# Da-Tsuchi/KLab_MultiModalModel

Hardware: AMD Instinct MI355X
Metric: caption-train samples/sec (224px img, 64-tok tgt) (higher is better)
Workload: dtype bf16; 1 GPU; BASELINE configs[1]: Swin-V2(C=64,(2,2,6,2),224,w7) frozen + T5-small, fwd+bwd+Adam, T5 dropout 0.1 on, random-init weights; global_batch=64, per_gpu_batch=64, src_len=9, tgt_len=64, parallelism=dp1, hipgraph=False, optimizer=klab.optim.FusedAdam (Adam update of ref/train.py:28, one kernel)

## Files before the change

include/klab_mm.h:

```cpp
#ifndef KLAB_MM_H
#define KLAB_MM_H
#include <stddef.h>
#include <stdint.h>

#ifdef __cplusplus
extern "C" {
#endif

#define KLAB_OK 0
#define KLAB_ERR_UNSUPPORTED (-2)
#define KLAB_ERR_BADARG (-3)

#define KLAB_F32 0
#define KLAB_BF16 1
#define KLAB_FP8 2

#define KLAB_ACT_NONE 0
#define KLAB_ACT_RELU 1
#define KLAB_ACT_GELU 2

#define KLAB_AUX_NONE 0
#define KLAB_AUX_NONZERO 1
#define KLAB_AUX_DGELU 2

// ... 54 lines not shown
                            int grp_stride, int off, float drop_p, const uint32_t* seed_dev, uint32_t tag, void* stream);

typedef struct klab_attn_args {
  int dtype;
  const void* q; long ldq;
  const void* k; long ldk;
  const void* v; long ldv;
  const float* bias; int causal;
  void* ctx; long ldo;
  float* lse;
  int B, H, Lq, Lk, dk;
  float drop_p; const uint32_t* seed_dev; uint32_t drop_tag;
  const void* dctx; long lddo;
  void* dq; long lddq;
  void* dk_out; long lddk;
  void* dv; long lddv;
  float* dbias;
  void* ds_ws;
  int ds_defer;
  const float* score_scale;
  int bias_mod;
} klab_attn_args;
int klab_t5_attn_fwd(const klab_attn_args* a, void* stream);
int klab_t5_attn_bwd(const klab_attn_args* a, void* stream);
typedef struct klab_attn_fused_args {
  const float* x; const float* gamma; float eps; int d_model;
  const void* w;
  void* xn; float* rstd;
  void* proj; long ldproj;
  int cross;
  klab_attn_args attn;
} klab_attn_fused_args;
int klab_t5_attn_fused_fwd(const klab_attn_fused_args* a, void* stream);
int klab_dbias_reduce(const void* ds_ws, int dtype, float* dbias, int nbatch, int H, int Lq, int Lk, void* stream);

typedef struct klab_swin_attn_args {
  int dtype;
  const void* qkv; void* ctx; const float* bias; const float* logit_scale; float* lse;
  int B, R, w, shift, H, C;
  const void* dctx; void* dqkv; float* dbias; float* dlogit_scale;
  void* bwd_ws; size_t bwd_ws_bytes;
  const float* bias_table; float* dbias_table;
  const float* v_bias; float* dv_bias;
} klab_swin_attn_args;
int klab_swin_attn_fwd(const klab_swin_attn_args* a, void* stream);
size_t klab_swin_attn_bwd_ws_bytes(int dtype, int B, int R, int w, int H, int C);
int klab_swin_qkv_attn_fused(const void* x, const void* wqkv, const float* bqkv, void* ctx, const float* bias, const float* logit_scale,
                             int dtype, int B, int R, int w, int shift, int H, int C, void* stream);
int klab_swin_attn_bwd(const klab_swin_attn_args* a, void* stream);
int klab_swin_cpb_bias(const float* coords, const int* index, const float* w0, const float* b0, const float* w2,
                       float* table, float* hidden, float* bias, int ntab, int n, int heads, int nhidden, void* stream);
int klab_swin_cpb_table(const float* coords, const float* w0, const float* b0, const float* w2, float* table, float* hidden,
                        float* bias_table, int ntab, int heads, int nhidden, void* stream);
int klab_swin_cpb_table_bwd(const float* dbias_table, const float* bias_table, const float* coords, const float* hidden, const float* w2,
                            float* dtable, float* dw0, float* db0, float* dw2, int ntab, int heads, int nhidden, void* stream);

typedef struct klab_image_desc { long long offset; int height, width; } klab_image_desc;
size_t klab_image_preprocess_ws_bytes(int n_images, int max_h, int mid);
int klab_image_preprocess(const unsigned char* src, const klab_image_desc* desc_dev, int n_images, int max_h, int max_w, int mid,
                          int out_size, int filter_a, int filter_b, double rescale, const float* mean3, const float* std3,
                          float* pixel_values, void* ws, size_t ws_bytes, void* stream);

#define KLAB_JPEG_GRAY 0
#define KLAB_JPEG_YCC 1
#define KLAB_JPEG_RGB 2
typedef struct klab_jpeg_info {
// ... 151 lines not shown
```

klab_multimodalmodel_amd/_lib.py:

```python
import ctypes as C
import os

HERE = os.path.dirname(os.path.abspath(__file__))
LIB_PATH = os.environ.get("KLAB_LIB", os.path.join(HERE, "libklab_mm.so"))

F32, BF16, FP8 = 0, 1, 2
ACT_NONE, ACT_RELU, ACT_GELU = 0, 1, 2
AUX_NONE, AUX_NONZERO, AUX_DGELU = 0, 1, 2
ERR_UNSUPPORTED, ERR_BADARG = -2, -3

vp, i32, i64, f32, u32 = C.c_void_p, C.c_int, C.c_long, C.c_float, C.c_uint32


class GemmArgs(C.Structure):
    _fields_ = [("M", i32), ("N", i32), ("K", i32), ("dtype", i32),
                ("A", vp), ("lda", i64), ("a_kmajor", i32),
                ("B", vp), ("ldb", i64), ("b_kmajor", i32),
                ("C", vp), ("ldc", i64), ("c_dtype", i32), ("accumulate", i32),
                ("alpha", f32), ("alpha_dev", vp), ("bias", vp), ("act", i32),
                ("aux", vp), ("ldaux", i64), ("aux_mode", i32), ("aux_scale", f32),
                ("residual", vp), ("ldr", i64), ("r_dtype", i32),
                ("drop_p", f32), ("seed_dev", vp), ("drop_tag", u32), ("name_tag", i32), ("atomic_ok", i32)]


class AttnArgs(C.Structure):
    _fields_ = [("dtype", i32), ("q", vp), ("ldq", i64), ("k", vp), ("ldk", i64), ("v", vp), ("ldv", i64),
                ("bias", vp), ("causal", i32), ("ctx", vp), ("ldo", i64), ("lse", vp),
                ("B", i32), ("H", i32), ("Lq", i32), ("Lk", i32), ("dk", i32),
                ("drop_p", f32), ("seed_dev", vp), ("drop_tag", u32),
                ("dctx", vp), ("lddo", i64), ("dq", vp), ("lddq", i64), ("dk_out", vp), ("lddk", i64),
                ("dv", vp), ("lddv", i64), ("dbias", vp), ("ds_ws", vp), ("ds_defer", i32),
                ("score_scale", vp), ("bias_mod", i32)]


class AttnFusedArgs(C.Structure):
    _fields_ = [("x", vp), ("gamma", vp), ("eps", f32), ("d_model", i32), ("w", vp), ("xn", vp), ("rstd", vp), ("proj", vp), ("ldproj", i64),
                ("cross", i32), ("attn", AttnArgs)]


class SwinAttnArgs(C.Structure):
    _fields_ = [("dtype", i32), ("qkv", vp), ("ctx", vp), ("bias", vp), ("logit_scale", vp), ("lse", vp),
                ("B", i32), ("R", i32), ("w", i32), ("shift", i32), ("H", i32), ("C", i32),
                ("dctx", vp), ("dqkv", vp), ("dbias", vp), ("dlogit_scale", vp),
                ("bwd_ws", vp), ("bwd_ws_bytes", C.c_size_t), ("bias_table", vp), ("dbias_table", vp),
                ("v_bias", vp), ("dv_bias", vp)]


class BeamUpdateArgs(C.Structure):
    _fields_ = [("B", i32), ("k", i32), ("V", i32), ("max_length", i32), ("eos_id", i32), ("early_stopping", i32), ("length_penalty", f32),
                ("cand_score", vp), ("cand_idx", vp), ("run_seq_in", vp), ("run_seq_out", vp), ("run_score", vp),
                ("fin_seq_in", vp), ("fin_seq_out", vp), ("fin_score", vp), ("fin_flag", vp), ("fin_len", vp), ("unsat", vp),
                ("slot_in", vp), ("slot_out", vp), ("prev_tokens", vp), ("parent", vp), ("stop_word", vp)]


SIGNATURES = {
    "klab_version": [],
    "klab_gemm": [C.POINTER(GemmArgs), vp],
    "klab_gemm_probe_enable": [i32],
    "klab_gemm_probe_read": [vp, vp, vp],
    "klab_rmsnorm_fwd": [vp, vp, vp, i32, vp, vp, i32, i32, f32, i32, i32, i32, f32, vp, u32, vp],
    "klab_rmsnorm_bwd": [vp, vp, vp, vp, vp, vp, vp, i32, vp, i32, i32, i32, i32, i32, f32, u32, f32, u32, vp, vp],
    "klab_rmsnorm_bwd_part": [vp, vp, vp, vp, vp, vp, vp, i32, vp, i32, i32, i32, i32, i32, f32, u32, f32, u32, vp, vp],
    "klab_rmsnorm_part_rows": [i32],
    "klab_colpart_reduce": [vp, i64, i32, i32, vp, i32, vp],
    "klab_adam_step": [vp, i32, i64, vp, vp, vp, vp, i32, f32, f32, f32, f32, f32, f32, f32, vp],
    "klab_adam_step_range": [vp, i32, i64, i64, vp, vp, vp, vp, i32, f32, f32, f32, f32, f32, f32, f32, vp],
    "klab_layernorm_fwd": [vp, i32, vp, vp, vp, vp, vp, i32, vp, vp, i32, i32, f32, i32, i32, i32, f32, vp, u32, vp],
    "klab_layernorm_bwd": [vp, vp, i32, vp, vp, vp, vp, vp, vp, i32, i32, i32, i32, i32, f32, vp, u32, vp],
    "klab_rmsnorm_fwd_q8": [vp, vp, vp, vp, vp, vp, i32, i32, f32, f32, vp, u32, vp],
    "klab_layernorm_fwd_q8": [vp, vp, vp, vp, vp, vp, vp, vp, vp, vp, i32, i32, f32, vp],
    "klab_gelu_fwd": [vp, vp, i32, i64, vp],
    "klab_gelu_fwd_q8": [vp, vp, vp, vp, i32, i32, vp],
    "klab_layernorm_bwd_bias": [vp, vp, i32, vp, vp, vp, vp, vp, vp, vp, i32, i32, i32, i32, i32, f32, vp, u32, vp],
    "klab_t5_attn_fwd": [C.POINTER(AttnArgs), vp],
    "klab_t5_attn_bwd": [C.POINTER(AttnArgs), vp],
    "klab_t5_attn_fused_fwd": [C.POINTER(AttnFusedArgs), vp],
    "klab_t5_decode_attn": [i32, vp, i64, vp, vp, i64, i64, vp, i64, vp, i64, i32, i32, i32, i32, vp],
    "klab_t5_beam_decode_attn": [i32, vp, i64, vp, vp, i64, i64, i32, vp, i64, vp, i64, vp, i64, i32, i32, i32, i32, vp],
    "klab_beam_topk": [i32, vp, i64, i32, vp, i32, i32, i32, vp, vp, vp, vp, vp],
    "klab_beam_update": [C.POINTER(BeamUpdateArgs), i32, vp],
    "klab_beam_init": [C.POINTER(BeamUpdateArgs), i32, i32, vp],
    "klab_beam_copy_rows": [i32, vp, i64, i32, vp, i64, i32, i32, vp],
    "klab_dbias_reduce": [vp, i32, vp, i32, i32, i32, i32, vp],
    "klab_swin_mlp_fused": [vp, vp, vp, vp, vp, vp, vp, vp, vp, vp, i32, i32, i32, f32, vp],
    "klab_gemm_grouped": [vp, i32, vp],
    "klab_gemm_fp8": [C.POINTER(GemmArgs), vp, vp, i64, vp],
    "klab_quant_fp8_rows": [vp, i64, i32, i32, vp, i64, vp, vp],
    "klab_quant_fp8_arena": [vp, i32, i64, vp, vp, vp, vp],
    "klab_swin_qkv_attn_fused": [vp, vp, vp, vp, vp, vp, i32, i32, i32, i32, i32, i32, i32, vp],
    "klab_swin_linear_ln_fused": [vp, vp, vp, vp, vp, vp, vp, vp, i32, i32, i32, i32, f32, vp],
    "klab_swin_patch_embed_fused": [vp, vp, i32, vp, vp, vp, vp, vp, i32, i32, i32, i32, i32, i32, f32, vp],
    "klab_swin_proj_ln_fused": [vp, vp, vp, vp, vp, vp, vp, vp, i32, i32, i32, f32, vp],
    "klab_swin_attn_fwd": [C.POINTER(SwinAttnArgs), vp],
    "klab_swin_attn_bwd": [C.POINTER(SwinAttnArgs), vp],
    "klab_swin_attn_bwd_ws_bytes": [i32, i32, i32, i32, i32, i32],
    "klab_swin_cpb_bias": [vp, vp, vp, vp, vp, vp, vp, vp, i32, i32, i32, i32, vp],
    "klab_swin_cpb_table": [vp, vp, vp, vp, vp, vp, vp, i32, i32, i32, vp],
    "klab_swin_cpb_table_bwd": [vp, vp, vp, vp, vp, vp, vp, vp, vp, i32, i32, i32, vp],
    "klab_cast_pack": [vp, i32, i64, vp, i32, vp],
    "klab_embed_fwd": [vp, i32, i32, i32, i32, vp, i32, vp, i32, i32, f32, vp, u32, vp, vp],
    "klab_embed_bwd": [vp, i32, i32, i32, i32, vp, vp, i32, i32, i32, f32, vp, u32, vp],
    "klab_relbias_fwd": [vp, vp, vp, i32, i32, i32, vp],
    "klab_relbias_bwd": [vp, vp, vp, i32, i32, i32, i32, vp],
    "klab_ce_fwd": [vp, i64, i32, vp, i32, i32, vp, vp, vp, i32, vp],
    "klab_ce_count": [vp, i32, vp, vp],
    "klab_im2col_patch": [vp, vp, i32, i32, i32, i32, i32, vp],
    "klab_im2col_patch_ld": [vp, vp, i32, i32, i32, i32, i32, i32, vp],
    "klab_merge_gather": [vp, vp, i32, i32, i32, i32, vp],
    "klab_merge_scatter": [vp, vp, i32, i32, i32, vp],
# ... 77 lines not shown
```

klab_multimodalmodel_amd/csrc/engine.cpp:

```cpp
#include <hip/hip_runtime.h>
#include <math.h>
#include <stdio.h>
#include <string.h>

#include <string>
#include <vector>

#include "gemm_shared.h"
#include "klab_mm.h"

namespace {

#define RC(x)                 \
  do {                        \
    int rc__ = (x);           \
    if (rc__ != 0) return rc__; \
  } while (0)

struct ParamInfo {
  std::string name;
  std::vector<long> shape;
  long numel = 0;
  long grad_off = -1;
  long warena_off = -1;
// ... 613 lines not shown
    e->q8_src[side] = a; e->q8_rows[side] = M; e->q8_k[side] = F;
    return 0;
  }
  return klab_gelu_fwd(z, a, c.dt, (long)M * F, c.ws());
}

int linear_fwd(const Ctx& c, const void* x, int M, int K, long woffv, int N, void* y, long ldy, int ydt, const float* bias = nullptr,
               int act = 0) {
  klab_gemm_args g = G0(c, M, N, K, x, K, 1, woff(c, woffv), K, 1, y, ldy, ydt);
  g.bias = bias; g.act = act;
  return fwd_gemm(c, g, woffv);
}
int linear_dgrad(const Ctx& c, const void* dy, long lddy, int M, int N, long woffv, int K, void* dx, int dxdt) {
  klab_gemm_args g = G0(c, M, K, N, dy, lddy, 1, woff(c, woffv), K, 0, dx, K, dxdt);
  return klab_gemm(&g, c.ws());
}
int linear_wgrad(const Ctx& c, const void* dy, long lddy, const void* x, long ldx, int M, int N, int K, float* dw) {
  klab_gemm_args g = G0(c, N, K, M, dy, lddy, 0, x, ldx, 0, dw, K, KLAB_F32);
  g.accumulate = 1; g.atomic_ok = 1;
  return klab_gemm(&g, c.ws());
}

int t5_sublayer_out(const Ctx& c, const void* x, int M, int K, long woffv, int d, const float* resid, float* hout, float p, uint32_t tag) {
  klab_gemm_args g = G0(c, M, d, K, x, K, 1, woff(c, woffv), K, 1, hout, d, KLAB_F32);
  g.residual = resid; g.ldr = d; g.r_dtype = KLAB_F32;
  g.drop_p = p; g.seed_dev = c.e->seed_dev; g.drop_tag = tag;
  return fwd_gemm(c, g, woffv);
}

static bool attn_fused_on() {
  static const bool on = [] { const char* v = getenv("KLAB_T5_ATTN_FUSED"); return !v || atoi(v) != 0; }();
  return on;
}

int t5_stack_forward(const Ctx& c, const klab_t5_cfg& cfg, const std::vector<ParamInfo>& P, const std::vector<const float*>& W,
                     const std::vector<T5LayerIdx>& L, int final_ln, T5StackBufs& s, bool dec, int stack_id, float p, int B,
                     const void* kv_all, int Lkv, long kv_ld, float* out_f32, int grp, int grp_stride, int off, float p_final) {
  const int d = cfg.d_model, H = cfg.n_heads, dk = cfg.d_kv, inner = H * dk, ff = cfg.d_ff;
  const int M = s.M, Lq = s.Lseq;
  const int relb = L[0].relb;
  if (c.e->bias_ready[stack_id]) c.e->bias_ready[stack_id] = false;
  else RC(klab_relbias_fwd(W[relb], s.bucket, s.bias, H, Lq, Lq, c.ws()));
  int j = 0;
  for (size_t i = 0; i < L.size(); ++i) {
    const T5LayerIdx& l = L[i];
    T5LayerBufs& b = s.L[i];
    {
      klab_attn_args a;
      memset(&a, 0, sizeof(a));
      a.dtype = c.dt; a.q = b.qkv; a.ldq = 3 * inner; a.k = eoff(c, b.qkv, inner); a.ldk = 3 * inner;
      a.v = eoff(c, b.qkv, 2 * inner); a.ldv = 3 * inner; a.bias = s.bias; a.causal = dec ? 1 : 0;
      a.ctx = b.ctx; a.ldo = inner; a.lse = b.lse; a.B = B; a.H = H; a.Lq = Lq; a.Lk = Lq; a.dk = dk;
      a.drop_p = p; a.seed_dev = c.e->seed_dev; a.drop_tag = tag_of(stack_id, (int)i, SITE_PROB);
      int frc = KLAB_ERR_UNSUPPORTED;
      if (attn_fused_on() && c.dt == KLAB_BF16 && !c.e->fp8 && Lq >= 32) {
        klab_attn_fused_args fa;
        memset(&fa, 0, sizeof(fa));
        fa.x = s.h[j]; fa.gamma = W[l.ln0]; fa.eps = cfg.ln_eps; fa.d_model = d; fa.w = woff(c, P[l.q].warena_off);
        fa.xn = b.xn1; fa.rstd = b.rstd1; fa.proj = b.qkv; fa.ldproj = 3 * inner; fa.cross = 0; fa.attn = a;
        frc = klab_t5_attn_fused_fwd(&fa, c.ws());
        if (frc != 0 && frc != KLAB_ERR_UNSUPPORTED) return frc;
      }
      if (frc != 0) {
        RC(rms_fwd_for_linear(c, s.h[j], W[l.ln0], b.xn1, b.rstd1, M, d, cfg.ln_eps));
        RC(linear_fwd(c, b.xn1, M, d, P[l.q].warena_off, 3 * inner, b.qkv, 3 * inner, c.dt));
        RC(klab_t5_attn_fwd(&a, c.ws()));
// ... 95 lines not shown
    q.clear();
    return 0;
  }
};

int t5_stack_backward(const Ctx& c, const klab_t5_cfg& cfg, const std::vector<ParamInfo>& P, const std::vector<const float*>& W,
                      float* Gflat, const std::vector<T5LayerIdx>& L, int final_ln, T5StackBufs& s, bool dec, int stack_id, float p,
                      int B, const void* kv_all, void* dkv_all, int Lkv, long kv_ld, float** dh_out) {
  klab_engine* e = c.e;
  const int d = cfg.d_model, H = cfg.n_heads, dk = cfg.d_kv, inner = H * dk, ff = cfg.d_ff;
  const int M = s.M, Lq = s.Lseq;
  const int nsub = dec ? 3 : 2;
  int j = nsub * (int)L.size();
  float* dh_cur = e->dh_a;
  float* dh_oth = e->dh_b;
  auto G = [&](int pi) { return Gflat + P[pi].grad_off; };
  const float inv_keep = p > 0.f ? 1.f / (1.f - p) : 1.f;
  int dy_i = 0, deferred = 0;
  WgradQueue wq;
  const int stk = dec ? 1 : 0;
  const bool part_ok = Gflat == e->G[2] && e->rms_part && d <= 1024 && (long)klab_rmsnorm_part_rows(M) * d <= e->rms_part_stride;
  int rms_calls = 0;
  auto rms_bwd = [&](const float* dyin, const float* x, const float* w, const float* rstd, const float* dres, float* dx, void* dxt, int pidx,
                     float p_y, uint32_t tag_y, float p_prev, uint32_t tag_prev) -> int {
    if (part_ok)
      return klab_rmsnorm_bwd_part(dyin, x, w, rstd, dres, dx, dxt, c.dt, e->rms_part + (long)(rms_calls++) * e->rms_part_stride, M, d, 0, 0, 0,
                                   p_y, tag_y, p_prev, tag_prev, e->seed_dev, c.ws());
    return klab_rmsnorm_bwd(dyin, x, w, rstd, dres, dx, dxt, c.dt, G(pidx), M, d, 0, 0, 0, p_y, tag_y, p_prev, tag_prev, e->seed_dev, c.ws());
  };
  auto next_dy = [&]() { return e->dy_pool[dy_i++ % e->dy_pool.size()]; };
  if (e->dbias_zeroed[stk]) e->dbias_zeroed[stk] = false;
  else RC(hipMemsetAsync(s.dbias, 0, (size_t)H * Lq * Lq * 4, c.s));
  void* dy = next_dy();
  RC(rms_bwd(e->dxn, s.h[j], W[final_ln], s.rstd_f, nullptr, dh_cur, dy, final_ln, p, tag_of(stack_id, 0, SITE_FINAL), p,
             tag_of(stack_id, (int)L.size() - 1, SITE_FFN_OUT)));
  std::vector<int> pending_buckets;
  const int Ln = (int)L.size();
  std::vector<char> flush_at(Ln, 1);
  static const int group_tiles = [] { const char* v = getenv("KLAB_WGRAD_GROUP_TILES"); return v ? atoi(v) : 90; }();
  static const bool kv_per_layer = [] { const char* v = getenv("KLAB_KV_WGRAD_PER_LAYER"); return !v || atoi(v) != 0; }();
  const bool kv_in_queue = dec && dkv_all && kv_per_layer && Gflat == e->G[2] && !e->use_graph && e->kvall_g_off >= 0;
  if (group_tiles > 0 && Ln >= 3 && Gflat == e->G[2] && !e->use_graph) {
    auto T2 = [](int n, int k) { return (long)((n + 255) / 256) * ((k + 255) / 256); };
    const long tl = T2(d, ff) + T2(ff, d) + T2(d, inner) + T2(3 * inner, d) + (dec ? T2(d, inner) + T2(inner, d) + (kv_in_queue ? T2(2 * inner, d) : 0) : 0);
    const int per_group = (int)((group_tiles + tl - 1) / tl), per_layer = dec ? 7 : 4;
    if (per_group >= 2) {
      const int body = Ln - 1;
      int ng = body / per_group;
      if (ng < 1) ng = 1;
      if (((body + ng - 1) / ng) * per_layer <= 32) {
        std::fill(flush_at.begin(), flush_at.end(), 0);
        int i = Ln - 1;
        for (int gi = 0; gi < ng; ++gi) { i -= body / ng + (gi < body % ng ? 1 : 0); flush_at[i + 1] = 1; }
        flush_at[0] = 1;
      }
    }
  }
  for (int i = (int)L.size() - 1; i >= 0; --i) {
    const T5LayerIdx& l = L[i];
    T5LayerBufs& b = s.L[i];
    void* dhmid = e->dhmid_pool[i];
    void* dqkv = e->dqkv_pool[i];
    --j;
    wq.push(dy, d, b.hmid, ff, M, d, ff, G(l.wo));
    {
      klab_gemm_args g = G0(c, M, ff, d, dy, d, 1, woff(c, P[l.wo].warena_off), ff, 0, dhmid, ff, c.dt);
      g.aux = b.hmid; g.ldaux = ff; g.aux_mode = KLAB_AUX_NONZERO; g.aux_scale = inv_keep;
      RC(klab_gemm(&g, c.ws()));
    }
    wq.push(dhmid, ff, b.xn3, d, M, ff, d, G(l.wi));
    RC(linear_dgrad(c, dhmid, ff, M, ff, P[l.wi].warena_off, d, e->dxn, KLAB_F32));
    {
      const uint32_t tprev = dec ? tag_of(stack_id, i, SITE_XOUT) : tag_of(stack_id, i, SITE_ATTN_OUT);
      dy = next_dy();
      RC(rms_bwd(e->dxn, s.h[j], W[l.ln2], b.rstd3, dh_cur, dh_oth, dy, l.ln2, 0.f, 0, p, tprev));
      float* t = dh_cur; dh_cur = dh_oth; dh_oth = t;
    }
    if (dec) {
      --j;
      void* dqc = e->dqc_pool[i];
      wq.push(dy, d, b.ctx2, inner, M, d, inner, G(l.co));
      RC(linear_dgrad(c, dy, d, M, d, P[l.co].warena_off, inner, e->dctx, c.dt));
      klab_attn_args a;
      memset(&a, 0, sizeof(a));
      a.dtype = c.dt; a.q = b.qc; a.ldq = inner;
      a.k = eoff(c, (void*)kv_all, (long)i * 2 * inner); a.ldk = kv_ld;
      a.v = eoff(c, (void*)kv_all, (long)i * 2 * inner + inner); a.ldv = kv_ld;
      a.ctx = b.ctx2; a.ldo = inner; a.lse = b.lse2; a.B = B; a.H = H; a.Lq = Lq; a.Lk = Lkv; a.dk = dk;
      a.drop_p = p; a.seed_dev = e->seed_dev; a.drop_tag = tag_of(stack_id, i, SITE_XPROB);
      a.dctx = e->dctx; a.lddo = inner; a.dq = dqc; a.lddq = inner;
      a.dk_out = eoff(c, dkv_all, (long)i * 2 * inner); a.lddk = kv_ld;
      a.dv = eoff(c, dkv_all, (long)i * 2 * inner + inner); a.lddv = kv_ld;
      RC(klab_t5_attn_bwd(&a, c.ws()));
      if (kv_in_queue) {
        wq.push(eoff(c, dkv_all, (long)i * 2 * inner), kv_ld, e->enc.out_t, d, B * Lkv, 2 * inner, d, Gflat + e->kvall_g_off + (long)i * 2 * inner * d);
        e->kv_wgrad_done = true;
      }
      wq.push(dqc, inner, b.xn2, d, M, inner, d, G(l.cq));
      RC(linear_dgrad(c, dqc, inner, M, inner, P[l.cq].warena_off, d, e->dxn, KLAB_F32));
      dy = next_dy();
      RC(rms_bwd(e->dxn, s.h[j], W[l.ln1], b.rstd2, dh_cur, dh_oth, dy, l.ln1, 0.f, 0, p, tag_of(stack_id, i, SITE_ATTN_OUT)));
      float* t = dh_cur; dh_cur = dh_oth; dh_oth = t;
    }
    --j;
    wq.push(dy, d, b.ctx, inner, M, d, inner, G(l.o));
    RC(linear_dgrad(c, dy, d, M, d, P[l.o].warena_off, inner, e->dctx, c.dt));
    {
      klab_attn_args a;
      memset(&a, 0, sizeof(a));
      a.dtype = c.dt; a.q = b.qkv; a.ldq = 3 * inner; a.k = eoff(c, b.qkv, inner); a.ldk = 3 * inner;
      a.v = eoff(c, b.qkv, 2 * inner); a.ldv = 3 * inner; a.bias = s.bias; a.causal = dec ? 1 : 0;
      a.ctx = b.ctx; a.ldo = inner; a.lse = b.lse; a.B = B; a.H = H; a.Lq = Lq; a.Lk = Lq; a.dk = dk;
      a.drop_p = p; a.seed_dev = e->seed_dev; a.drop_tag = tag_of(stack_id, i, SITE_PROB);
      a.dctx = e->dctx; a.lddo = inner; a.dq = dqkv; a.lddq = 3 * inner;
      a.dk_out = eoff(c, dqkv, inner); a.lddk = 3 * inner; a.dv = eoff(c, dqkv, 2 * inner); a.lddv = 3 * inner;
      a.dbias = s.dbias;
      int arc = KLAB_ERR_UNSUPPORTED;
      if (c.dt == KLAB_BF16 && deferred == (int)L.size() - 1 - i) {
        a.ds_defer = 1;
        a.ds_ws = (char*)e->ds_ws + (size_t)deferred * B * H * Lq * ((Lq + 31) & ~31) * c.es;
        arc = klab_t5_attn_bwd(&a, c.ws());
        if (arc == 0) ++deferred;
      }
      if (arc == KLAB_ERR_UNSUPPORTED) { a.ds_defer = 0; a.ds_ws = nullptr; arc = klab_t5_attn_bwd(&a, c.ws()); }
      RC(arc);
    }
    wq.push(dqkv, 3 * inner, b.xn1, d, M, 3 * inner, d, G(l.q));
    RC(linear_dgrad(c, dqkv, 3 * inner, M, 3 * inner, P[l.q].warena_off, d, e->dxn, KLAB_F32));
    {
      const bool first = (i == 0);
      if (!first) dy = next_dy();
      RC(rms_bwd(e->dxn, s.h[j], W[l.ln0], b.rstd1, dh_cur, dh_oth, first ? nullptr : dy, l.ln0, 0.f, 0, first ? 0.f : p,
                 first ? 0u : tag_of(stack_id, i - 1, SITE_FFN_OUT)));
      float* t = dh_cur; dh_cur = dh_oth; dh_oth = t;
    }
    bool launched = false;
    RC(wq.flush(c, flush_at[i] != 0, &launched));
    pending_buckets.push_back((int)L.size() - 1 - i);
    if (launched) {
      const int seg = dec ? 0 : 1;
      for (int bi : pending_buckets)
        if (e->bucket_events_on && Gflat == e->G[2] && !e->use_graph && bi < (int)e->bucket_ev[seg].size())
          RC((int)hipEventRecord(e->bucket_ev[seg][bi], e->side));
      pending_buckets.clear();
      if (i == 0 && e->bucket_events_on && Gflat == e->G[2] && !e->use_graph && (int)L.size() - 1 < (int)e->bucket_ev[seg].size())
        e->bucket_ev_live[seg] = true;
    }
  }
  if (part_ok && rms_calls) {
    if (rms_calls != e->rms_ncalls[stk]) return KLAB_ERR_BADARG;
    RC(klab_colpart_reduce(e->rms_part, e->rms_part_stride, klab_rmsnorm_part_rows(M), d, e->rms_dst_dev[stk], rms_calls, c.ws()));
  }
  if (deferred) RC(klab_dbias_reduce(e->ds_ws, c.dt, s.dbias, deferred * B, H, Lq, Lq, c.ws()));
  RC(klab_relbias_bwd(s.dbias, s.bucket, G(L[0].relb), H, Lq, Lq, cfg.rel_buckets, c.ws()));
  *dh_out = dh_cur;
  return 0;
}
// ... 1091 lines not shown
```

klab_multimodalmodel_amd/ops.py:

```python
import ctypes as C

import torch

from . import _lib as L


def _seed_ptr(seed):
    return None if seed is None else seed.data_ptr()


def gemm(A, B, C_out, *, M, N, K, a_kmajor=True, b_kmajor=True, lda=None, ldb=None, ldc=None, alpha=1.0,
         alpha_dev=None, bias=None, act=L.ACT_NONE, aux=None, aux_mode=L.AUX_NONE, aux_scale=1.0, residual=None,
         drop_p=0.0, seed=None, tag=0, accumulate=False, atomic_ok=False, name_tag=0):
    lib = L.load()
    a = L.GemmArgs()
    a.atomic_ok, a.name_tag = int(atomic_ok), name_tag
    a.M, a.N, a.K = M, N, K
    a.dtype = L.dtype_code(A.dtype)
    assert B.dtype == A.dtype
    a.A, a.lda, a.a_kmajor = A.data_ptr(), (lda if lda is not None else A.stride(0)), int(a_kmajor)
    a.B, a.ldb, a.b_kmajor = B.data_ptr(), (ldb if ldb is not None else B.stride(0)), int(b_kmajor)
    a.C, a.ldc, a.c_dtype = C_out.data_ptr(), (ldc if ldc is not None else C_out.stride(0)), L.dtype_code(C_out.dtype)
    a.accumulate = int(accumulate)
    a.alpha = alpha
# ... 160 lines not shown
def swin_patch_embed_fused(pixels, w_padded, bias, gamma, beta, out, outt, *, patch=4, eps=1e-5):
    lib = L.load()
    B, cin, H, _ = pixels.shape
    L.check(lib.klab_swin_patch_embed_fused(pixels.data_ptr(), w_padded.data_ptr(), w_padded.stride(0), bias.data_ptr(), gamma.data_ptr(),
                                            beta.data_ptr(), out.data_ptr(), L.ptr(outt), L.dtype_code(w_padded.dtype), B, cin, H, patch,
                                            out.shape[1], eps, L.stream_ptr()), "klab_swin_patch_embed_fused")


def t5_attn_fused_fwd(x, gamma, w, xn, rstd, proj, ctx, lse, *, B, H, Lq, Lk, dk, eps=1e-6, bias=None, causal=False, cross=False, k=None, v=None,
                      ldk=None, ldv=None, drop_p=0.0, seed=None, tag=0):
    lib = L.load()
    fa = L.AttnFusedArgs()
    fa.x, fa.gamma, fa.eps, fa.d_model = x.data_ptr(), gamma.data_ptr(), eps, x.shape[1]
    fa.w, fa.xn, fa.rstd, fa.proj, fa.ldproj, fa.cross = w.data_ptr(), xn.data_ptr(), rstd.data_ptr(), proj.data_ptr(), proj.stride(0), int(cross)
    kk, vv = (k, v) if cross else (proj, proj)
    fa.attn = _attn_args(proj, kk, vv, ctx, lse, bias, causal, B, H, Lq, Lk, dk, drop_p, seed, tag, proj.stride(0),
                         ldk or kk.stride(0), ldv or vv.stride(0), ctx.stride(0))
    L.check(lib.klab_t5_attn_fused_fwd(C.byref(fa), L.stream_ptr()), "klab_t5_attn_fused_fwd")


def t5_attn_bwd(q, k, v, ctx, lse, dctx, dq, dk_out, dv, *, B, H, Lq, Lk, dk, bias=None, causal=False, dbias=None,
                drop_p=0.0, seed=None, tag=0, ldq=None, ldk=None, ldv=None, ldo=None, lddo=None, lddq=None, lddk=None,
                lddv=None, ds_ws=None):
    lib = L.load()
    a = _attn_args(q, k, v, ctx, lse, bias, causal, B, H, Lq, Lk, dk, drop_p, seed, tag,
                   ldq or q.stride(0), ldk or k.stride(0), ldv or v.stride(0), ldo or ctx.stride(0))
    a.dctx, a.lddo = dctx.data_ptr(), lddo or dctx.stride(0)
    a.dq, a.lddq = dq.data_ptr(), lddq or dq.stride(0)
    a.dk_out, a.lddk = dk_out.data_ptr(), lddk or dk_out.stride(0)
    a.dv, a.lddv = dv.data_ptr(), lddv or dv.stride(0)
    a.dbias = L.ptr(dbias)
    a.ds_ws = L.ptr(ds_ws)
    L.check(lib.klab_t5_attn_bwd(C.byref(a), L.stream_ptr()), "klab_t5_attn_bwd")


def _swin_args(qkv, ctx, bias, logit_scale, lse, B, R, w, shift, H, Cc, bias_table=None, v_bias=None, dv_bias=None):
    a = L.SwinAttnArgs()
    a.v_bias, a.dv_bias = L.ptr(v_bias), L.ptr(dv_bias)
    a.dtype = L.dtype_code(qkv.dtype)
    a.qkv, a.ctx, a.bias, a.logit_scale, a.lse = qkv.data_ptr(), ctx.data_ptr(), L.ptr(bias), logit_scale.data_ptr(), L.ptr(lse)
    a.bias_table = L.ptr(bias_table)
    a.B, a.R, a.w, a.shift, a.H, a.C = B, R, w, shift, H, Cc
    return a


def swin_attn_fwd(qkv, ctx, bias, logit_scale, lse=None, *, B, R, w, shift, H, C, bias_table=None, mfma=True, v_bias=None):
    import torch
    lib = L.load()
    a = _swin_args(qkv, ctx, bias, logit_scale, lse, B, R, w, shift, H, C, bias_table, v_bias)
    if mfma and (w * w > 64 or R % w):
        nbytes = lib.klab_swin_attn_bwd_ws_bytes(a.dtype, B, R, w, H, C)
        if nbytes:
            ws = torch.empty(nbytes, dtype=torch.uint8, device=qkv.device)
            a.bwd_ws, a.bwd_ws_bytes = ws.data_ptr(), nbytes
    L.check(lib.klab_swin_attn_fwd(C_byref(a), L.stream_ptr()), "klab_swin_attn_fwd")


def swin_attn_bwd(qkv, ctx, bias, logit_scale, lse, dctx, dqkv, dbias=None, dlogit_scale=None, *, B, R, w, shift, H, C, mfma=True,
                  bias_table=None, dbias_table=None, v_bias=None, dv_bias=None):
    import torch
    lib = L.load()
    a = _swin_args(qkv, ctx, bias, logit_scale, lse, B, R, w, shift, H, C, bias_table, v_bias, dv_bias)
    a.dbias_table = L.ptr(dbias_table)
    a.dctx, a.dqkv, a.dbias, a.dlogit_scale = dctx.data_ptr(), dqkv.data_ptr(), L.ptr(dbias), L.ptr(dlogit_scale)
    nbytes = lib.klab_swin_attn_bwd_ws_bytes(a.dtype, B, R, w, H, C) if mfma else 0
    if nbytes:
# ... 244 lines not shown
```

Measured before the change: 11360 samples/s.

## Fuse output-projection dgrad into T5 attention backward kernel

Adds a fused HIP kernel that computes the attention-output gradient (dy times the output-projection weight slice for each head) in LDS via MFMA, then runs the attention backward (dS, dQ, dK, dV) in the same block. This removes the separate linear_dgrad GEMM and the round-trip of dctx through global memory for the T5 decoder self- and cross-attention. In exchange, each (batch, head) block reloads its 512x64 weight slice and the full dy rows, and the kernel only handles d_model=512, dk=64 and Lq, Lk up to 64. Other shapes fall back to the old two-call path.

```diff
diff --git a/include/klab_mm.h b/include/klab_mm.h
--- a/include/klab_mm.h
+++ b/include/klab_mm.h
@@ -110,6 +110,13 @@
   klab_attn_args attn;
 } klab_attn_fused_args;
 int klab_t5_attn_fused_fwd(const klab_attn_fused_args* a, void* stream);
+typedef struct klab_attn_bwd_fused_args {
+  const void* dy; long lddy;
+  const void* w;
+  int d_model;
+  klab_attn_args attn;
+} klab_attn_bwd_fused_args;
+int klab_t5_attn_bwd_fused(const klab_attn_bwd_fused_args* a, void* stream);
 int klab_dbias_reduce(const void* ds_ws, int dtype, float* dbias, int nbatch, int H, int Lq, int Lk, void* stream);
 
 typedef struct klab_swin_attn_args {
diff --git a/klab_multimodalmodel_amd/_lib.py b/klab_multimodalmodel_amd/_lib.py
--- a/klab_multimodalmodel_amd/_lib.py
+++ b/klab_multimodalmodel_amd/_lib.py
@@ -38,6 +38,10 @@
                 ("cross", i32), ("attn", AttnArgs)]
 
 
+class AttnBwdFusedArgs(C.Structure):
+    _fields_ = [("dy", vp), ("lddy", i64), ("w", vp), ("d_model", i32), ("attn", AttnArgs)]
+
+
 class SwinAttnArgs(C.Structure):
     _fields_ = [("dtype", i32), ("qkv", vp), ("ctx", vp), ("bias", vp), ("logit_scale", vp), ("lse", vp),
                 ("B", i32), ("R", i32), ("w", i32), ("shift", i32), ("H", i32), ("C", i32),
@@ -75,6 +79,7 @@
     "klab_t5_attn_fwd": [C.POINTER(AttnArgs), vp],
     "klab_t5_attn_bwd": [C.POINTER(AttnArgs), vp],
     "klab_t5_attn_fused_fwd": [C.POINTER(AttnFusedArgs), vp],
+    "klab_t5_attn_bwd_fused": [C.POINTER(AttnBwdFusedArgs), vp],
     "klab_t5_decode_attn": [i32, vp, i64, vp, vp, i64, i64, vp, i64, vp, i64, i32, i32, i32, i32, vp],
     "klab_t5_beam_decode_attn": [i32, vp, i64, vp, vp, i64, i64, i32, vp, i64, vp, i64, vp, i64, i32, i32, i32, i32, vp],
     "klab_beam_topk": [i32, vp, i64, i32, vp, i32, i32, i32, vp, vp, vp, vp, vp],
diff --git a/klab_multimodalmodel_amd/csrc/attn_t5_bwd_fused.hip b/klab_multimodalmodel_amd/csrc/attn_t5_bwd_fused.hip
--- /dev/null
+++ b/klab_multimodalmodel_amd/csrc/attn_t5_bwd_fused.hip
@@ -0,0 +1,297 @@
+#include <math.h>
+#include <stdlib.h>
+#include <string.h>
+
+#include "common.h"
+#include "klab_mm.h"
+
+namespace klab {
+
+int dbias_reduce_dispatch(const void* ds_ws, float* dbias, int nbatch, int H, int Lq, int Lk, hipStream_t s);
+
+namespace abf {
+
+constexpr int D = 512, DK = 64, KT = 64, NKT = D / KT, SLOT = 16384, NSLOT = 2, NBUF = 3;
+constexpr int PITCHB = 160, GROUPB = 8 * PITCHB + 128, IMG = 8 * GROUPB;
+__device__ __forceinline__ int off(int row, int col) { return (row >> 3) * GROUPB + (row & 7) * PITCHB + col * 2; }
+
+typedef __attribute__((address_space(3))) bf16x4 lds_bf16x4_t;
+__device__ __forceinline__ bf16x4 tr4(const char* p) { return __builtin_amdgcn_ds_read_tr16_b64_v4bf16((lds_bf16x4_t*)p); }
+
+__device__ __forceinline__ bf16x8 tr_frag(const char* img, int row0, int col0, int lane) {
+  const int g = lane >> 4, q4 = (lane & 15) >> 2, pp = lane & 3;
+  const int r = row0 + 4 * g + q4;
+  const bf16x4 lo = tr4(img + off(r, col0 + 4 * pp)), hi = tr4(img + off(r + 16, col0 + 4 * pp));
+  return bf16x8{lo[0], lo[1], lo[2], lo[3], hi[0], hi[1], hi[2], hi[3]};
+}
+__device__ __forceinline__ bf16x8 row_frag(const char* img, int r, int ks, int lane) {
+  return *reinterpret_cast<const bf16x8*>(img + off(r, ks * 32 + (lane >> 4) * 8));
+}
+__device__ __forceinline__ bf16x8 pack8(const f32x4& a, const f32x4& b) {
+  return bf16x8{(bf16_t)a[0], (bf16_t)a[1], (bf16_t)a[2], (bf16_t)a[3], (bf16_t)b[0], (bf16_t)b[1], (bf16_t)b[2], (bf16_t)b[3]};
+}
+
+struct P {
+  const bf16_t* dy; long lddy;
+  const bf16_t* w;
+  const bf16_t* q; long ldq; const bf16_t* k; long ldk; const bf16_t* v; long ldv;
+  const bf16_t* ctx; long ldo; const float* lse;
+  const float* bias; int causal;
+  int B, H, Lq, Lk;
+  float p; const uint32_t* seed; uint32_t tag;
+  bf16_t* dq; long lddq; bf16_t* dkk; long lddk; bf16_t* dv; long lddv;
+  float* dbias; bf16_t* ds_ws;
+};
+
+__global__ __launch_bounds__(256, 2) void t5_attn_bwd_fused(P p) {
+  extern __shared__ __attribute__((aligned(16))) char smem[];
+  char* Qi = smem;
+  char* Ki = Qi + IMG;
+  char* Vi = Ki + IMG;
+  char* dOi = Vi + IMG;
+  char* ring = dOi + IMG;
+  char* PDi = ring;
+  char* dSi = ring + IMG;
+  const int Lq = p.Lq, Lk = p.Lk, H = p.H;
+  int b, h;
+  {
+    const int i = blockIdx.x;
+    if ((p.B & 7) == 0) { const int xcd = i & 7, kk = i >> 3; h = kk % H; b = (kk / H) * 8 + xcd; }
+    else { b = i / H; h = i % H; }
+  }
+  const int tid = threadIdx.x, lane = tid & 63;
+  const int wave = __builtin_amdgcn_readfirstlane(tid >> 6);
+  const int g = lane >> 4;
+  const int q0 = wave * 16, q = q0 + (lane & 15), qc = q < Lq ? q : Lq - 1;
+
+  const bf16_t* wsrc[2];
+  const bf16_t* dysrc[2];
+#pragma unroll
+  for (int u = 0; u < 2; ++u) {
+    const int r = (tid + u * 256) >> 3, c = tid & 7;
+    wsrc[u] = p.w + (long)r * D + h * DK + c * 8;
+    dysrc[u] = p.dy + ((long)b * Lq + (r < Lq ? r : Lq - 1)) * p.lddy + c * 8;
+  }
+  bf16x8 rw[NBUF][2], rd[NBUF][2];
+  auto load_tile = [&](int kt, int sb) {
+#pragma unroll
+    for (int u = 0; u < 2; ++u) {
+      rw[sb][u] = *reinterpret_cast<const bf16x8*>(wsrc[u] + (long)kt * KT * D);
+      rd[sb][u] = *reinterpret_cast<const bf16x8*>(dysrc[u] + kt * KT);
+    }
+  };
+  auto store_tile = [&](int sb, char* st) {
+#pragma unroll
+    for (int u = 0; u < 2; ++u) {
+      const int r = (tid + u * 256) >> 3, pos = ((tid & 7) ^ (r & 7)) * 16;
+      *reinterpret_cast<bf16x8*>(st + r * 128 + pos) = rw[sb][u];
+      *reinterpret_cast<bf16x8*>(st + 8192 + r * 128 + pos) = rd[sb][u];
+    }
+  };
+
+  bf16x8 vq[2], vk[2], vv[2];
+#pragma unroll
+  for (int u = 0; u < 2; ++u) {
+    const int ch = tid + u * 256, r = ch >> 3, c = (ch & 7) * 8;
+    vq[u] = bf16x8{}; vk[u] = bf16x8{}; vv[u] = bf16x8{};
+    if (r < Lq) vq[u] = *reinterpret_cast<const bf16x8*>(p.q + ((long)b * Lq + r) * p.ldq + h * DK + c);
+    if (r < Lk) {
+      vk[u] = *reinterpret_cast<const bf16x8*>(p.k + ((long)b * Lk + r) * p.ldk + h * DK + c);
+      vv[u] = *reinterpret_cast<const bf16x8*>(p.v + ((long)b * Lk + r) * p.ldv + h * DK + c);
+    }
+  }
+  f32x4 bv[4];
+  {
+    const float* brow = p.bias ? p.bias + ((long)h * Lq + qc) * Lk : nullptr;
+#pragma unroll
+    for (int t = 0; t < 4; ++t)
+#pragma unroll
+      for (int r = 0; r < 4; ++r) {
+        const int key = t * 16 + g * 4 + r;
+        bv[t][r] = brow ? brow[key < Lk ? key : Lk - 1] : 0.f;
+      }
+  }
+  const float lq = q < Lq ? p.lse[((long)b * H + h) * Lq + q] : INFINITY;
+  bf16x4 ov[4];
+#pragma unroll
+  for (int jt = 0; jt < 4; ++jt) ov[jt] = *reinterpret_cast<const bf16x4*>(p.ctx + ((long)b * Lq + qc) * p.ldo + h * DK + jt * 16 + g * 4);
+#pragma unroll
+  for (int i = 0; i < NBUF; ++i) load_tile(i, i);
+#pragma unroll
+  for (int u = 0; u < 2; ++u) {
+    const int ch = tid + u * 256, r = ch >> 3, c = (ch & 7) * 8;
+    *reinterpret_cast<bf16x8*>(Qi + off(r, c)) = vq[u];
+    *reinterpret_cast<bf16x8*>(Ki + off(r, c)) = vk[u];
+    *reinterpret_cast<bf16x8*>(Vi + off(r, c)) = vv[u];
+  }
+
+  f32x4 acc[4];
+#pragma unroll
+  for (int jt = 0; jt < 4; ++jt) acc[jt] = f32x4{0.f, 0.f, 0.f, 0.f};
+  {
+    const int q4 = (lane & 15) >> 2, pp = lane & 3;
+    const int ql = wave * 16 + (lane & 15);
+#pragma unroll
+    for (int kt = 0; kt < NKT; ++kt) {
+      char* st = ring + (kt & 1) * SLOT;
+      store_tile(kt % NBUF, st);
+      if (kt + NBUF < NKT) load_tile(kt + NBUF, kt % NBUF);
+      asm volatile("s_waitcnt lgkmcnt(0)" ::: "memory");
+      __builtin_amdgcn_s_barrier();
+      const char* Ws = st;
+      const char* Ds = st + 8192;
+#pragma unroll
+      for (int ks = 0; ks < 2; ++ks) {
+        const int c0 = 4 * ks + (g >> 1);
+        const bf16x4 dlo = *reinterpret_cast<const bf16x4*>(Ds + ql * 128 + ((c0 ^ (ql & 7)) * 16) + (g & 1) * 8);
+        const bf16x4 dhi = *reinterpret_cast<const bf16x4*>(Ds + ql * 128 + (((c0 + 2) ^ (ql & 7)) * 16) + (g & 1) * 8);
+        const bf16x8 dyf = bf16x8{dlo[0], dlo[1], dlo[2], dlo[3], dhi[0], dhi[1], dhi[2], dhi[3]};
+        const int r = ks * 32 + 4 * g + q4;
+#pragma unroll
+        for (int jt = 0; jt < 4; ++jt) {
+          const int chunk = 2 * jt + (pp >> 1);
+          const bf16x4 lo = tr4(Ws + r * 128 + ((chunk ^ (r & 7)) * 16) + (pp & 1) * 8);
+          const bf16x4 hi = tr4(Ws + (r + 16) * 128 + ((chunk ^ (r & 7)) * 16) + (pp & 1) * 8);
+          const bf16x8 wf = bf16x8{lo[0], lo[1], lo[2], lo[3], hi[0], hi[1], hi[2], hi[3]};
+          acc[jt] = __builtin_amdgcn_mfma_f32_16x16x32_bf16(wf, dyf, acc[jt], 0, 0, 0);
+        }
+      }
+    }
+  }
+  float delta;
+  {
+    float a = 0.f;
+#pragma unroll
+    for (int jt = 0; jt < 4; ++jt) {
+      bf16x4 o = bf16x4{(bf16_t)acc[jt][0], (bf16_t)acc[jt][1], (bf16_t)acc[jt][2], (bf16_t)acc[jt][3]};
+      if (q >= Lq) o = bf16x4{};
+#pragma unroll
+      for (int r = 0; r < 4; ++r) a += (float)o[r] * (float)ov[jt][r];
+      *reinterpret_cast<bf16x4*>(dOi + off(q, jt * 16 + g * 4)) = o;
+    }
+    a += __shfl_xor(a, 16, 64);
+    a += __shfl_xor(a, 32, 64);
+    delta = a;
+  }
+  __syncthreads();
+
+  const DropCtx dc = drop_slab(make_drop(p.seed, p.tag, p.p), (uint32_t)(b * H + h));
+  const int Lkp = (Lk + 31) & ~31, NS = Lkp / 32;
+  {
+    bf16x8 qf[2], dof[2];
+#pragma unroll
+    for (int ks = 0; ks < 2; ++ks) { qf[ks] = row_frag(Qi, q, ks, lane); dof[ks] = row_frag(dOi, q, ks, lane); }
+    float* dbrow = (p.dbias && !p.ds_ws && q < Lq) ? p.dbias + ((long)h * Lq + q) * Lk : nullptr;
+    bf16_t* dsrow = (p.ds_ws && q < Lq) ? p.ds_ws + (((long)b * H + h) * Lq + q) * Lkp : nullptr;
+    f32x4 dqa[4];
+#pragma unroll
+    for (int dt = 0; dt < 4; ++dt) dqa[dt] = f32x4{0.f, 0.f, 0.f, 0.f};
+#pragma unroll
+    for (int sidx = 0; sidx < 2; ++sidx) {
+      if (sidx < NS) {
+        f32x4 pd2[2], ds2[2];
+#pragma unroll
+        for (int u = 0; u < 2; ++u) {
+          const int t = 2 * sidx + u;
+          f32x4 st = {0.f, 0.f, 0.f, 0.f}, dpt = {0.f, 0.f, 0.f, 0.f};
+#pragma unroll
+          for (int ks = 0; ks < 2; ++ks) {
+            st = __builtin_amdgcn_mfma_f32_16x16x32_bf16(row_frag(Ki, t * 16 + (lane & 15), ks, lane), qf[ks], st, 0, 0, 0);
+            dpt = __builtin_amdgcn_mfma_f32_16x16x32_bf16(row_frag(Vi, t * 16 + (lane & 15), ks, lane), dof[ks], dpt, 0, 0, 0);
+          }
+#pragma unroll
+          for (int r = 0; r < 4; ++r) {
+            const int key = t * 16 + g * 4 + r;
+            const bool ok = key < Lk && q < Lq && !(p.causal && key > q);
+            const float pr = ok ? __expf(st[r] + bv[t][r] - lq) : 0.f;
+            const float mlt = drop_mult32_nb(dc, (uint32_t)q * (uint32_t)Lk + key);
+            const float dsv = pr * (dpt[r] * mlt - delta);
+            if (dbrow) { if (ok) atomicAdd(dbrow + key, dsv); }
+            pd2[u][r] = pr * mlt;
+            ds2[u][r] = dsv;
+          }
+        }
+        const bf16x8 pdf = pack8(pd2[0], pd2[1]), dsf = pack8(ds2[0], ds2[1]);
+        const bf16x4 ds_lo = bf16x4{dsf[0], dsf[1], dsf[2], dsf[3]}, ds_hi = bf16x4{dsf[4], dsf[5], dsf[6], dsf[7]};
+        *reinterpret_cast<bf16x4*>(PDi + off(q, sidx * 32 + g * 4)) = bf16x4{pdf[0], pdf[1], pdf[2], pdf[3]};
+        *reinterpret_cast<bf16x4*>(PDi + off(q, sidx * 32 + 16 + g * 4)) = bf16x4{pdf[4], pdf[5], pdf[6], pdf[7]};
+        *reinterpret_cast<bf16x4*>(dSi + off(q, sidx * 32 + g * 4)) = ds_lo;
+        *reinterpret_cast<bf16x4*>(dSi + off(q, sidx * 32 + 16 + g * 4)) = ds_hi;
+        if (dsrow) {
+          *reinterpret_cast<bf16x4*>(dsrow + sidx * 32 + g * 4) = ds_lo;
+          *reinterpret_cast<bf16x4*>(dsrow + sidx * 32 + 16 + g * 4) = ds_hi;
+        }
+#pragma unroll
+        for (int dt = 0; dt < 4; ++dt) dqa[dt] = __builtin_amdgcn_mfma_f32_16x16x32_bf16(tr_frag(Ki, sidx * 32, dt * 16, lane), dsf, dqa[dt], 0, 0, 0);
+      }
+    }
+    if (q < Lq) {
+#pragma unroll
+      for (int dt = 0; dt < 4; ++dt)
+        *reinterpret_cast<bf16x4*>(p.dq + ((long)b * Lq + q) * p.lddq + h * DK + dt * 16 + g * 4) =
+            bf16x4{(bf16_t)dqa[dt][0], (bf16_t)dqa[dt][1], (bf16_t)dqa[dt][2], (bf16_t)dqa[dt][3]};
+    }
+  }
+  __syncthreads();
+
+  const int k0 = wave * 16;
+  if (k0 >= Lk) return;
+  const int NQS = (Lq + 31) / 32;
+  f32x4 av[4], ak[4];
+#pragma unroll
+  for (int dt = 0; dt < 4; ++dt) { av[dt] = f32x4{0.f, 0.f, 0.f, 0.f}; ak[dt] = f32x4{0.f, 0.f, 0.f, 0.f}; }
+#pragma unroll
+  for (int sidx = 0; sidx < 2; ++sidx) {
+    if (sidx < NQS) {
+      const bf16x8 pf = tr_frag(PDi, sidx * 32, k0, lane), sf = tr_frag(dSi, sidx * 32, k0, lane);
+#pragma unroll
+      for (int dt = 0; dt < 4; ++dt) {
+        av[dt] = __builtin_amdgcn_mfma_f32_16x16x32_bf16(tr_frag(dOi, sidx * 32, dt * 16, lane), pf, av[dt], 0, 0, 0);
+        ak[dt] = __builtin_amdgcn_mfma_f32_16x16x32_bf16(tr_frag(Qi, sidx * 32, dt * 16, lane), sf, ak[dt], 0, 0, 0);
+      }
+    }
+  }
+  const int key = k0 + (lane & 15);
+  if (key < Lk) {
+#pragma unroll
+    for (int dt = 0; dt < 4; ++dt) {
+      const int dd = h * DK + dt * 16 + g * 4;
+      *reinterpret_cast<bf16x4*>(p.dv + ((long)b * Lk + key) * p.lddv + dd) = bf16x4{(bf16_t)av[dt][0], (bf16_t)av[dt][1], (bf16_t)av[dt][2], (bf16_t)av[dt][3]};
+      *reinterpret_cast<bf16x4*>(p.dkk + ((long)b * Lk + key) * p.lddk + dd) = bf16x4{(bf16_t)ak[dt][0], (bf16_t)ak[dt][1], (bf16_t)ak[dt][2], (bf16_t)ak[dt][3]};
+    }
+  }
+}
+
+}
+}
+
+using namespace klab;
+
+extern "C" int klab_t5_attn_bwd_fused(const klab_attn_bwd_fused_args* fb, void* stream) {
+  if (!fb) return KLAB_ERR_BADARG;
+  const klab_attn_args* a = &fb->attn;
+  if (!fb->dy || !fb->w || !a->q || !a->k || !a->v || !a->ctx || !a->lse || !a->dq || !a->dk_out || !a->dv) return KLAB_ERR_BADARG;
+  if (a->B <= 0) return KLAB_OK;
+  if (a->dtype != KLAB_BF16 || fb->d_model != abf::D || a->dk != abf::DK || a->H * a->dk != abf::D) return KLAB_ERR_UNSUPPORTED;
+  if (a->Lq < 1 || a->Lq > 64 || a->Lk < 1 || a->Lk > 64 || a->score_scale || a->bias_mod) return KLAB_ERR_UNSUPPORTED;
+  auto al = [](const void* p, long ld, int elems) { return ((uintptr_t)p % (elems * 2)) == 0 && ld % elems == 0; };
+  if (!al(fb->dy, fb->lddy, 8) || fb->lddy < abf::D || !al(fb->w, 0, 8) || !al(a->q, a->ldq, 8) || !al(a->k, a->ldk, 8) ||
+      !al(a->v, a->ldv, 8) || !al(a->ctx, a->ldo, 4) || !al(a->dq, a->lddq, 4) || !al(a->dk_out, a->lddk, 4) || !al(a->dv, a->lddv, 4))
+    return KLAB_ERR_UNSUPPORTED;
+  if (a->ds_ws && ((uintptr_t)a->ds_ws & 7)) return KLAB_ERR_UNSUPPORTED;
+  abf::P p;
+  p.dy = (const bf16_t*)fb->dy; p.lddy = fb->lddy; p.w = (const bf16_t*)fb->w;
+  p.q = (const bf16_t*)a->q; p.ldq = a->ldq; p.k = (const bf16_t*)a->k; p.ldk = a->ldk; p.v = (const bf16_t*)a->v; p.ldv = a->ldv;
+  p.ctx = (const bf16_t*)a->ctx; p.ldo = a->ldo; p.lse = a->lse; p.bias = a->bias; p.causal = a->causal;
+  p.B = a->B; p.H = a->H; p.Lq = a->Lq; p.Lk = a->Lk; p.p = a->drop_p; p.seed = a->seed_dev; p.tag = a->drop_tag;
+  p.dq = (bf16_t*)a->dq; p.lddq = a->lddq; p.dkk = (bf16_t*)a->dk_out; p.lddk = a->lddk; p.dv = (bf16_t*)a->dv; p.lddv = a->lddv;
+  p.dbias = a->dbias; p.ds_ws = (bf16_t*)a->ds_ws;
+  hipStream_t s = (hipStream_t)stream;
+  const size_t lds = 4 * (size_t)abf::IMG + abf::NSLOT * (size_t)abf::SLOT;
+  int rc = ensure_dyn_lds(reinterpret_cast<const void*>(abf::t5_attn_bwd_fused), lds);
+  if (rc) return rc;
+  hipLaunchKernelGGL(abf::t5_attn_bwd_fused, dim3(a->B * a->H), dim3(256), lds, s, p);
+  KLAB_LAUNCH_CHECK();
+  if (a->dbias && a->ds_ws && !a->ds_defer) return dbias_reduce_dispatch(a->ds_ws, a->dbias, a->B, a->H, a->Lq, a->Lk, s);
+  return KLAB_OK;
+}
diff --git a/klab_multimodalmodel_amd/csrc/engine.cpp b/klab_multimodalmodel_amd/csrc/engine.cpp
--- a/klab_multimodalmodel_amd/csrc/engine.cpp
+++ b/klab_multimodalmodel_amd/csrc/engine.cpp
@@ -669,6 +669,10 @@
   static const bool on = [] { const char* v = getenv("KLAB_T5_ATTN_FUSED"); return !v || atoi(v) != 0; }();
   return on;
 }
+static bool attn_bwd_fused_on() {
+  static const bool on = [] { const char* v = getenv("KLAB_T5_ATTN_BWD_FUSED"); return !v || atoi(v) != 0; }();
+  return on;
+}
 
 int t5_stack_forward(const Ctx& c, const klab_t5_cfg& cfg, const std::vector<ParamInfo>& P, const std::vector<const float*>& W,
                      const std::vector<T5LayerIdx>& L, int final_ln, T5StackBufs& s, bool dec, int stack_id, float p, int B,
@@ -830,6 +834,18 @@
   if (e->dbias_zeroed[stk]) e->dbias_zeroed[stk] = false;
   else RC(hipMemsetAsync(s.dbias, 0, (size_t)H * Lq * Lq * 4, c.s));
   void* dy = next_dy();
+  bool dctx_ready = false;
+  auto attn_bwd = [&](klab_attn_args& a, long wo_off) -> int {
+    if (attn_bwd_fused_on() && c.dt == KLAB_BF16) {
+      klab_attn_bwd_fused_args fb;
+      memset(&fb, 0, sizeof(fb));
+      fb.dy = dy; fb.lddy = d; fb.w = woff(c, wo_off); fb.d_model = d; fb.attn = a;
+      const int frc = klab_t5_attn_bwd_fused(&fb, c.ws());
+      if (frc != KLAB_ERR_UNSUPPORTED) return frc;
+    }
+    if (!dctx_ready) { RC(linear_dgrad(c, dy, d, M, d, wo_off, inner, e->dctx, c.dt)); dctx_ready = true; }
+    return klab_t5_attn_bwd(&a, c.ws());
+  };
   RC(rms_bwd(e->dxn, s.h[j], W[final_ln], s.rstd_f, nullptr, dh_cur, dy, final_ln, p, tag_of(stack_id, 0, SITE_FINAL), p,
              tag_of(stack_id, (int)L.size() - 1, SITE_FFN_OUT)));
   std::vector<int> pending_buckets;
@@ -878,7 +894,7 @@
       --j;
       void* dqc = e->dqc_pool[i];
       wq.push(dy, d, b.ctx2, inner, M, d, inner, G(l.co));
-      RC(linear_dgrad(c, dy, d, M, d, P[l.co].warena_off, inner, e->dctx, c.dt));
+      dctx_ready = false;
       klab_attn_args a;
       memset(&a, 0, sizeof(a));
       a.dtype = c.dt; a.q = b.qc; a.ldq = inner;
@@ -889,7 +905,7 @@
       a.dctx = e->dctx; a.lddo = inner; a.dq = dqc; a.lddq = inner;
       a.dk_out = eoff(c, dkv_all, (long)i * 2 * inner); a.lddk = kv_ld;
       a.dv = eoff(c, dkv_all, (long)i * 2 * inner + inner); a.lddv = kv_ld;
-      RC(klab_t5_attn_bwd(&a, c.ws()));
+      RC(attn_bwd(a, P[l.co].warena_off));
       if (kv_in_queue) {
         wq.push(eoff(c, dkv_all, (long)i * 2 * inner), kv_ld, e->enc.out_t, d, B * Lkv, 2 * inner, d, Gflat + e->kvall_g_off + (long)i * 2 * inner * d);
         e->kv_wgrad_done = true;
@@ -902,7 +918,7 @@
     }
     --j;
     wq.push(dy, d, b.ctx, inner, M, d, inner, G(l.o));
-    RC(linear_dgrad(c, dy, d, M, d, P[l.o].warena_off, inner, e->dctx, c.dt));
+    dctx_ready = false;
     {
       klab_attn_args a;
       memset(&a, 0, sizeof(a));
@@ -917,10 +933,10 @@
       if (c.dt == KLAB_BF16 && deferred == (int)L.size() - 1 - i) {
         a.ds_defer = 1;
         a.ds_ws = (char*)e->ds_ws + (size_t)deferred * B * H * Lq * ((Lq + 31) & ~31) * c.es;
-        arc = klab_t5_attn_bwd(&a, c.ws());
+        arc = attn_bwd(a, P[l.o].warena_off);
         if (arc == 0) ++deferred;
       }
-      if (arc == KLAB_ERR_UNSUPPORTED) { a.ds_defer = 0; a.ds_ws = nullptr; arc = klab_t5_attn_bwd(&a, c.ws()); }
+      if (arc == KLAB_ERR_UNSUPPORTED) { a.ds_defer = 0; a.ds_ws = nullptr; arc = attn_bwd(a, P[l.o].warena_off); }
       RC(arc);
     }
     wq.push(dqkv, 3 * inner, b.xn1, d, M, 3 * inner, d, G(l.q));
diff --git a/klab_multimodalmodel_amd/ops.py b/klab_multimodalmodel_amd/ops.py
--- a/klab_multimodalmodel_amd/ops.py
+++ b/klab_multimodalmodel_amd/ops.py
@@ -216,6 +216,21 @@
     a.dbias = L.ptr(dbias)
     a.ds_ws = L.ptr(ds_ws)
     L.check(lib.klab_t5_attn_bwd(C.byref(a), L.stream_ptr()), "klab_t5_attn_bwd")
+
+
+def t5_attn_bwd_fused(dy, w, q, k, v, ctx, lse, dq, dk_out, dv, *, B, H, Lq, Lk, dk, bias=None, causal=False, dbias=None, ds_ws=None,
+                      ds_defer=False, drop_p=0.0, seed=None, tag=0, ldq=None, ldk=None, ldv=None, ldo=None, lddq=None, lddk=None, lddv=None):
+    lib = L.load()
+    fb = L.AttnBwdFusedArgs()
+    fb.dy, fb.lddy, fb.w, fb.d_model = dy.data_ptr(), dy.stride(0), w.data_ptr(), dy.shape[1]
+    a = _attn_args(q, k, v, ctx, lse, bias, causal, B, H, Lq, Lk, dk, drop_p, seed, tag,
+                   ldq or q.stride(0), ldk or k.stride(0), ldv or v.stride(0), ldo or ctx.stride(0))
+    a.dq, a.lddq = dq.data_ptr(), lddq or dq.stride(0)
+    a.dk_out, a.lddk = dk_out.data_ptr(), lddk or dk_out.stride(0)
+    a.dv, a.lddv = dv.data_ptr(), lddv or dv.stride(0)
+    a.dbias, a.ds_ws, a.ds_defer = L.ptr(dbias), L.ptr(ds_ws), int(ds_defer)
+    fb.attn = a
+    L.check(lib.klab_t5_attn_bwd_fused(C.byref(fb), L.stream_ptr()), "klab_t5_attn_bwd_fused")
 
 
 def _swin_args(qkv, ctx, bias, logit_scale, lse, B, R, w, shift, H, Cc, bias_table=None, v_bias=None, dv_bias=None):
```

Measured after the change: 11630 samples/s, median of 6. 1.02x the previous value.
